# geometrian/simple-spectral

Hardware: AMD Instinct MI355X
Metric: Msamples/s (w*h*spp/s) cornell-srgb 512x512 (higher is better)
Workload: dtype f32

## Files before the change

### simple_spectral_amd/csrc/ssx_api.hip

```cpp
#include "ssx_kernels.hip"
#include "ssx_debug.hip"

#include "../../include/ssx.h"

#include <chrono>
#include <array>
#include <atomic>
#include <cstdarg>
#include <cstdio>
#include <cstdlib>
#include <cmath>
#include <algorithm>
#include <cstring>
#include <mutex>
#include <string>
#include <thread>
#include <vector>

#include <limits.h>
#include <set>

#include "ssx_jit.h"

namespace {
// ... 40 lines not shown
	int n_cus = 0;
	hipStream_t stream = nullptr;
	DeviceBuffer d_blob;
	uint32_t blob_words = 0;
	uint32_t path_blob_words = 0;
	uint32_t topology = 0;
	int jit_mode = SSX_JIT_BACKGROUND;
	const ssx_jit::Kernels* jit_kernels[ssx_jit::kVariants] = {};
	uint32_t libm = SSX_LIBM_BUILD;
	uint32_t variant = SSX_LIBM_BUILD;
	bool jit_pending = false, jit_requested = false;
	ssx_jit::VidTable jit_vid;
	DeviceBuffer d_blob_jit; uint32_t blob_jit_words = 0, path_blob_jit_words = 0;
	uint64_t generic_samples = 0;
	int jit_state = SSX_JIT_STATE_NONE; std::string jit_message;
	std::vector<DeviceBuffer> d_textures;
	DeviceBuffer d_jh_data;
	bool rgb_mode = false;
	bool fuse_resolve = true;
	float calib_frames = 0.0f;
	float calib_left = 0.0f;
	bool pre_hits = false;
	DeviceBuffer d_accum;
	DeviceBuffer d_unit_counter;
	int resident_blocks = 0;
	int gen_blocks = 0;
	uint32_t max_wave_slots = 0;
	uint32_t queue_words = SSX_QUEUE_WORDS_WIDE;
	DeviceBuffer d_samples;
	DeviceBuffer d_logs;
	DeviceBuffer d_out;
	DeviceBuffer d_peer;
	bool have_scene = false;
	bool have_cam_dir = false;

	std::thread worker;
	std::atomic<int> rendering{0};
	std::atomic<int> stop_flag{0};
	std::atomic<uint32_t> done_spp{0};
	std::atomic<uint32_t> done_tiles{0};
	uint32_t total_spp = 0;
	int worker_rc = 0;
	std::atomic<uint64_t> units_enqueued{0};
	ssx_render_params cur{};
	struct SumsState { bool continuable = false, noise_valid = false, spectral_valid = false; uint32_t noise_batches = 0; } sums;
	uint32_t k_begin = 0;
	uint64_t scene_digest = 0;
// ... 66 lines not shown

uint32_t tiles_across(uint32_t pixels) { return (pixels + 7u) / 8u; }
size_t accum_bytes(uint32_t width, uint32_t height) { return (size_t)tiles_across(width) * tiles_across(height) * 64u * 4 * sizeof(double); }
size_t image_bytes(uint32_t width, uint32_t height) { return (size_t)width * height * 4 * sizeof(float); }

SsxPixelGrid pixel_grid(const ssx_render_params* p) {
	const uint32_t tx = tiles_across(p->width);
	return SsxPixelGrid{ p->width, p->height, tx, p->tile_first, p->tile_stride, p->tile_skew % tx };
}
dim3 pixel_blocks(const ssx_render_params* p) { return dim3((p->width * p->height + 255u) / 256u); }

int clear_sums(ssx_ctx* ctx, uint32_t width, uint32_t height, hipStream_t stream) {
	SSX_HIP(ctx, hipMemsetAsync(ctx->d_accum.ptr, 0, accum_bytes(width, height), stream));
	return SSX_OK;
}
void sums_invalidate(ssx_ctx* ctx) { ctx->sums = ssx_ctx::SumsState{}; }
void sums_publish(ssx_ctx* ctx, uint32_t done_spp, int64_t noise_batches = -1) {
	if (noise_batches >= 0) { ctx->sums.noise_valid = true; ctx->sums.noise_batches = (uint32_t)noise_batches; }
	ctx->done_spp.store(done_spp); ctx->sums.continuable = true;
}

constexpr size_t kSampleBufferBudget = (size_t)16 << 30;
size_t bytes_per_sample(const ssx_ctx* ctx) { return ctx->spectral_bins ? SSX_BYTES_PER_SAMPLE_FLUX : SSX_BYTES_PER_SAMPLE; }
constexpr size_t kAuxWordsPer64Records = 5;
size_t bytes_per_64_records(const ssx_ctx* ctx) { return 64u * bytes_per_sample(ctx) + kAuxWordsPer64Records * sizeof(uint32_t); }
size_t sample_bytes(const ssx_ctx* ctx, size_t records) { return records / 64u * bytes_per_64_records(ctx); }
size_t sample_slots(const ssx_ctx* ctx) { return ctx->d_samples.bytes / bytes_per_64_records(ctx) * 64u; }
size_t log_records(const ssx_ctx* ctx) { return ctx->d_logs.bytes / SSX_LOG_BYTES_PER_RECORD; }
constexpr uint32_t kMinUnits = 3072;
constexpr uint64_t kSamplesPerSync = (uint64_t)32 << 20;

struct LaunchPlan { SsxKernelArgs args; uint32_t max_spp_per_launch; };

LaunchPlan make_plan(ssx_ctx* ctx, const ssx_render_params* p, bool ask_device = true) {
	LaunchPlan pl{};
	SsxKernelArgs& a = pl.args;
	a.blob = ctx->d_blob.as<uint32_t>(); a.blob_words = ctx->path_blob_words;
	a.width = p->width; a.height = p->height;
	a.inv_width = 1.0 / (double)p->width; a.inv_height = 1.0 / (double)p->height;
	a.tiles_x = tiles_across(p->width);
	a.n_tiles = a.tiles_x * tiles_across(p->height);
	a.tile_first = p->tile_first; a.tile_stride = p->tile_stride; a.tile_skew = p->tile_skew % a.tiles_x;
	a.indirect_only = p->indirect_only ? 1u : 0u;
	a.no_els = p->no_explicit_light_sampling ? 1u : 0u;
	a.no_flat_field = p->no_flat_field_correction ? 1u : 0u;
	a.seed = p->seed;
	a.rgb_mode = ctx->rgb_mode ? 1u : 0u;
	a.fuse_resolve = ctx->fuse_resolve ? 1u : 0u;
	a.pre_hits = ctx->pre_hits ? 1u : 0u;
	a.my_tiles = a.n_tiles > p->tile_first ? (a.n_tiles - p->tile_first + p->tile_stride - 1u) / p->tile_stride : 0u;
// ... 59 lines not shown
			ctx->stage_ms[k] += ms;
		}
	}
	ctx->ev_used = 0;
	return SSX_OK;
}

int timing_events(ssx_ctx* ctx, hipEvent_t** out) {
	if (ctx->ev_used + 6 > 6 * 64) { int r = collect_timing(ctx); if (r) return r; }
	while (ctx->ev_pool.size() < ctx->ev_used + 6) {
		hipEvent_t e;
		SSX_HIP(ctx, hipEventCreateWithFlags(&e, hipEventDisableSystemFence));
		ctx->ev_pool.push_back(e);
	}
	*out = &ctx->ev_pool[ctx->ev_used];
	ctx->ev_used += 6;
	return SSX_OK;
}

struct Batch { SsxKernelArgs a; uint32_t units; uint64_t n_rec; hipEvent_t* tev; int rc; };

uint32_t unit_spp_of(const ssx_ctx* ctx) { return ctx->calib_frames >= 2.0f ? SSX_MAX_UNIT_KS / 2u : SSX_MAX_UNIT_KS; }

Batch make_batch(ssx_ctx* ctx, const LaunchPlan& pl, uint32_t k0, uint32_t k1) {
	Batch b{};
	b.a = pl.args;
	SsxKernelArgs& a = b.a;
	const uint32_t n_k = k1 - k0;
	a.k0 = k0; a.k1 = k1;
	a.n_records = (uint64_t)a.my_tiles * n_k * 64u;
	uint32_t g = unit_spp_of(ctx);
	while (g > 1u && (uint64_t)((n_k + g - 1u) / g) * a.my_tiles < kMinUnits) g >>= 1;
	a.group_spp = g;
	if (a.group_spp > n_k) a.group_spp = n_k;
	a.unit_cohorts = (a.group_spp + SSX_COHORT_KS - 1u) / SSX_COHORT_KS;
	a.unit_grab = ctx->calib_frames >= 2.0f ? 1u : 4u;
	if (a.unit_grab < 1u || a.unit_grab > 32u || a.group_spp == 0u || a.unit_cohorts == 0u) {
		b.rc = fail(ctx, SSX_ERR_STATE, fmt("internal: launch with unit_grab = %u (1..32), group_spp = %u, unit_cohorts = %u", a.unit_grab, a.group_spp, a.unit_cohorts));
		return b;
	}
	a.n_groups = (n_k + a.group_spp - 1) / a.group_spp;
	b.units = a.my_tiles * a.n_groups;
	b.n_rec = a.n_records;
	b.rc = ensure_logs(ctx, a.unit_cohorts);
	if (b.rc == SSX_OK) bind_arrays(a, ctx->d_samples.as<uint8_t>(), a.n_records, ctx->d_logs.as<uint8_t>(), log_records(ctx), ctx->spectral_bins != 0u);
	a.accum = ctx->d_accum.as<double>();
	uint32_t* const aux = reinterpret_cast<uint32_t*>(ctx->d_samples.as<uint8_t>() + sample_slots(ctx) * bytes_per_sample(ctx));
	a.unit_state = aux;
	a.tile_mask = aux + b.units;
	if (b.rc == SSX_OK && (size_t)a.my_tiles * 4u + b.units > (sample_slots(ctx) / 64u) * kAuxWordsPer64Records) b.rc = fail(ctx, SSX_ERR_STATE, "internal: launch larger than the sample allocation");
	return b;
}

size_t path_lds_bytes(uint32_t blob_words, uint32_t queue_words) {
	size_t n = ((size_t)blob_words + SSX_LDS_PREFIX_WORDS) * 4 + 4u * ((size_t)SSX_QUEUE_ENTRIES * queue_words + SSX_WAVE_COUNTER_WORDS) * 4u;
#ifdef SSX_REGTIME
	n += 4u * SSX_NTIME * 8u;
#endif
	return n;
}
struct PathKernel { const char* name; void (*host)(SsxKernelArgs); };
#define SSX_PK(k) { #k, k }
static const PathKernel kPathKernels[ssx_jit::kVariants][3][2] = {
	{ { SSX_PK(ssx_render_kernel), SSX_PK(ssx_render_kernel_nq) }, { SSX_PK(ssx_render_kernel_cornell), SSX_PK(ssx_render_kernel_cornell_nq) },
	  { SSX_PK(ssx_render_kernel_plane), SSX_PK(ssx_render_kernel_plane_nq) } },
	{ { SSX_PK(ssx_render_kernel_glibc), SSX_PK(ssx_render_kernel_nq_glibc) }, { SSX_PK(ssx_render_kernel_cornell_glibc), SSX_PK(ssx_render_kernel_cornell_nq_glibc) },
	  { SSX_PK(ssx_render_kernel_plane_glibc), SSX_PK(ssx_render_kernel_plane_nq_glibc) } },
	{ { SSX_PK(ssx_render_kernel_flux), SSX_PK(ssx_render_kernel_nq_flux) }, { SSX_PK(ssx_render_kernel_cornell_flux), SSX_PK(ssx_render_kernel_cornell_nq_flux) },
	  { SSX_PK(ssx_render_kernel_plane_flux), SSX_PK(ssx_render_kernel_plane_nq_flux) } } };
#undef SSX_PK
static const char* const kJitKernelNames[2] = { "ssx_render_kernel_jit", "ssx_render_kernel_jit_nq" };
const PathKernel& path_kernel_of(const ssx_ctx* ctx, bool narrow) { return kPathKernels[ctx->variant][ctx->topology < 3u ? ctx->topology : 0u][narrow]; }
// ... 25 lines not shown
	} else {
		void* args[] = { &a };
		SSX_HIP(ctx, hipLaunchKernel(k.host, dim3(blocks), dim3(256), args, lds, stream));
	}
	return SSX_OK;
}
int pick_queue(ssx_ctx* ctx, uint32_t blob_words, uint32_t* queue_words, int* blocks_per_cu) {
	int wide = 0, narrow = 0, rc;
	if (path_lds_bytes(blob_words, SSX_QUEUE_WORDS_WIDE) <= 65536u)
		if ((rc = occupancy_of(ctx, path_kernel_ref(ctx, false), path_lds_bytes(blob_words, SSX_QUEUE_WORDS_WIDE), &wide))) return rc;
	if ((rc = occupancy_of(ctx, path_kernel_ref(ctx, true), path_lds_bytes(blob_words, SSX_QUEUE_WORDS_NARROW), &narrow))) return rc;
	const bool use_narrow = narrow > wide || env_on("SSX_NARROW_QUEUE");
	*queue_words = use_narrow ? SSX_QUEUE_WORDS_NARROW : SSX_QUEUE_WORDS_WIDE;
	if (blocks_per_cu) *blocks_per_cu = use_narrow ? narrow : wide;
	return SSX_OK;
}

bool fuses_generate(const ssx_ctx* ctx, const SsxKernelArgs& a) {
	const char* fuse_env = debug_env("SSX_FUSE_GEN");
	const bool tiles_fit = a.tiles_x <= 0xFFFFu && tiles_across(a.height) <= 0xFFFFu;
	return ctx->topology == 2u && !a.pre_hits && tiles_fit && !(fuse_env && fuse_env[0] == '0');
}

int enqueue_generate(ssx_ctx* ctx, const Batch& b, hipStream_t stream) {
	SsxKernelArgs ga = b.a;
	ga.blob_words = ctx->blob_words;
	if (ga.pre_hits) {
		hipLaunchKernelGGL(ssx_tile_mask_kernel, dim3((ga.my_tiles + 3u) / 4u), dim3(256), 0, stream, ga);
		SSX_HIP(ctx, hipGetLastError());
	}
	const KernelRef gen_kernel{ (const void*)ssx_generate_kernel };
	const size_t gen_lds = ((size_t)ga.blob_words + SSX_LDS_PREFIX_WORDS) * 4;
	if (ctx->gen_blocks == 0) { const int rc = blocks_that_fit(ctx, gen_kernel, gen_lds, &ctx->gen_blocks); if (rc) return rc; }
	const uint64_t want = (b.n_rec + 255u) / 256u;
	return launch_kernel(ctx, gen_kernel, (uint32_t)(want < (uint64_t)ctx->gen_blocks ? want : (uint64_t)ctx->gen_blocks), gen_lds, stream, ga);
}

int enqueue_path(ssx_ctx* ctx, Batch& b, const KernelRef& kernel, uint32_t queue_words, uint32_t blob_words, int resident_blocks, hipStream_t stream) {
	if (!ctx->d_unit_counter.ptr) {
		SSX_HIP(ctx, ctx->d_unit_counter.reserve(4 * sizeof(uint32_t)));
		SSX_HIP(ctx, hipMemsetAsync(ctx->d_unit_counter.ptr, 0, 4 * sizeof(uint32_t), stream));
	}
	b.a.blob_words = blob_words; b.a.queue_words = queue_words;
	SSX_HIP(ctx, hipMemsetAsync(ctx->d_unit_counter.ptr, 0, 2 * sizeof(uint32_t), stream));
	SSX_HIP(ctx, hipMemsetAsync(b.a.unit_state, 0, (size_t)b.units * sizeof(uint32_t), stream));
	b.a.unit_counter = ctx->d_unit_counter.as<uint32_t>();
	const uint32_t want_blocks = (b.units + 3u) / 4u;
	uint32_t blocks = want_blocks < (uint32_t)resident_blocks ? want_blocks : (uint32_t)resident_blocks;
	if (blocks * 4u > ctx->max_wave_slots) blocks = ctx->max_wave_slots / 4u;
	return launch_kernel(ctx, kernel, blocks, path_lds_bytes(blob_words, queue_words), stream, b.a);
}

int launch_batch(ssx_ctx* ctx, Batch& b, hipStream_t stream) {
	if (b.rc) return b.rc;
	int rc;
	if (ctx->timing) { if ((rc = timing_events(ctx, &b.tev))) return rc; SSX_HIP(ctx, hipEventRecord(b.tev[0], stream)); }
	b.a.fuse_gen = fuses_generate(ctx, b.a) ? 1u : 0u;
	if (!b.a.fuse_gen && (rc = enqueue_generate(ctx, b, stream))) return rc;
	if (ctx->timing) SSX_HIP(ctx, hipEventRecord(b.tev[1], stream));
	const bool plan = ctx->resident_blocks == 0;
	if (plan && (rc = pick_queue(ctx, b.a.blob_words, &ctx->queue_words, nullptr))) return rc;
	const KernelRef path_kernel = path_kernel_ref(ctx, ctx->queue_words == SSX_QUEUE_WORDS_NARROW);
	if (plan && (rc = blocks_that_fit(ctx, path_kernel, path_lds_bytes(b.a.blob_words, ctx->queue_words), &ctx->resident_blocks))) return rc;
	if ((rc = enqueue_path(ctx, b, path_kernel, ctx->queue_words, b.a.blob_words, ctx->resident_blocks, stream))) return rc;
	ctx->units_enqueued.fetch_add(b.units);
	if (ctx->timing) for (int k = 2; k < 6; ++k) SSX_HIP(ctx, hipEventRecord(b.tev[k], stream));
	return SSX_OK;
}

constexpr uint64_t kJitAfterSamples = kSamplesPerSync;
void maybe_swap_jit(ssx_ctx* ctx, uint64_t samples) {
	if (!ctx->jit_pending) return;
	std::string err;
	const ssx_jit::Kernels* k = nullptr;
	const ssx_jit::State st = ssx_jit::lookup(ctx->device, ctx->jit_vid, &k, &err, ctx->variant);
	if (st == ssx_jit::State::Ready) {
		std::swap(ctx->d_blob, ctx->d_blob_jit);
		ctx->blob_words = ctx->blob_jit_words; ctx->path_blob_words = ctx->path_blob_jit_words;
		ctx->topology = 3u;
		ctx->jit_kernels[ctx->variant] = k;
		ctx->resident_blocks = 0; ctx->gen_blocks = 0;
		ctx->jit_pending = false; ctx->jit_state = SSX_JIT_STATE_SPECIALISED;
	} else if (st == ssx_jit::State::Failed) {
		ctx->jit_pending = false; ctx->jit_state = SSX_JIT_STATE_FAILED; ctx->jit_message = err;
	} else {
		ctx->generic_samples += samples;
		if (!ctx->jit_requested && ctx->generic_samples >= kJitAfterSamples) { ssx_jit::request(ctx->jit_vid, ctx->variant); ctx->jit_requested = true; }
	}
}

int ensure_libm_kernels(ssx_ctx* ctx, uint32_t libm) {
	const ssx_jit::Kernels*& have = ctx->jit_kernels[libm];
	if (ctx->topology != 3u || have) return SSX_OK;
	std::string err;
	const ssx_jit::Kernels* k = ssx_jit::get(ctx->device, ctx->jit_vid, &err, libm);
	if (!k) return fail(ctx, SSX_ERR_STATE, "the scene's specialised kernels for this libm could not be compiled: " + err);
	have = k;
	return SSX_OK;
}

int ready_to_launch(ssx_ctx* ctx, const ssx_render_params* p, bool need_out) {
	const uint32_t variant = (ctx->spectral_bins && p->libm == SSX_LIBM_BUILD && !ctx->rgb_mode) ? ssx_jit::kVariantFlux : p->libm;
	const int rc = ensure_libm_kernels(ctx, variant);
	if (rc) return rc;
// ... 20 lines not shown

int calibrate(ssx_ctx* ctx) {
	ssx_render_params cp{};
	cp.struct_size = sizeof cp; cp.width = 64; cp.height = 64; cp.spp = 4; cp.tile_stride = 1;
	ctx->fuse_resolve = false;
	ctx->pre_hits = false;
	LaunchPlan pl = make_plan(ctx, &cp);
	int rc = ensure_samples(ctx, pl, cp.spp);
	if (rc) return rc;
	Batch b = make_batch(ctx, pl, 0, cp.spp);
	if (b.rc) return b.rc;
	if ((rc = enqueue_generate(ctx, b, ctx->stream))) return rc;
	const KernelRef kernel{ (const void*)ssx_calibrate_kernel };
	int blocks = 0;
	if ((rc = blocks_that_fit(ctx, kernel, path_lds_bytes(ctx->blob_words, SSX_QUEUE_WORDS_NARROW), &blocks))) return rc;
	if ((rc = enqueue_path(ctx, b, kernel, SSX_QUEUE_WORDS_NARROW, ctx->blob_words, blocks, ctx->stream))) return rc;
	SSX_HIP(ctx, hipStreamSynchronize(ctx->stream));
	std::vector<uint4> recs((size_t)b.n_rec);
	SSX_HIP(ctx, hipMemcpy(recs.data(), b.a.st, recs.size() * sizeof(uint4), hipMemcpyDeviceToHost));
	uint64_t frames = 0;
	for (const uint4& r : recs) frames += (r.y >> 2) & 0xFu;
	ctx->calib_frames = (float)((double)frames / (double)recs.size());
	uint32_t counters[2] = { 0u, 0u };
	SSX_HIP(ctx, hipMemcpy(counters, ctx->d_unit_counter.ptr, sizeof counters, hipMemcpyDeviceToHost));
	ctx->calib_left = (float)((double)counters[1] / (double)recs.size());
	ctx->pre_hits = ctx->calib_left >= 0.3f;
	if (const char* e = debug_env("SSX_PRE_HITS")) { if (e[0] != '\0') ctx->pre_hits = e[0] != '0'; }
	ctx->fuse_resolve = true;
	return ensure_logs(ctx, (unit_spp_of(ctx) + SSX_COHORT_KS - 1u) / SSX_COHORT_KS);
}

int launch_finalize(ssx_ctx* ctx, const ssx_render_params* p, uint32_t spp, float* d_out, hipStream_t stream, uint32_t done_tiles = 0xFFFFFFFFu) {
	hipLaunchKernelGGL(ssx_finalize_kernel, pixel_blocks(p), dim3(256), 0, stream,
	                   ctx->d_accum.as<const double>(), (float4*)d_out, pixel_grid(p), spp, ctx->rgb_mode ? 1u : 0u, done_tiles);
	SSX_HIP(ctx, hipGetLastError());
	return SSX_OK;
}

int noise_begin(ssx_ctx* ctx, const ssx_render_params* p, uint32_t k_begin, bool continuing);
int noise_batch(ssx_ctx* ctx, const ssx_render_params* p, uint32_t n_k, hipStream_t stream);
int spectral_refuses(ssx_ctx* ctx, const ssx_render_params& p, bool tile_walk);
int spectral_begin(ssx_ctx* ctx, uint32_t my_tiles, bool continuing, bool* active);
int spectral_batch(ssx_ctx* ctx, const ssx_render_params* p, const LaunchPlan& pl, uint32_t n_k, hipStream_t stream);

int finish_walk(ssx_ctx* ctx, const ssx_render_params& p, uint32_t spp, uint32_t done_tiles) {
	if (const int rc = launch_finalize(ctx, &p, spp, ctx->d_out.as<float>(), ctx->stream, done_tiles)) return rc;
	SSX_HIP(ctx, hipStreamSynchronize(ctx->stream));
// ... 314 lines not shown
	if (ctx->jit_pending) {
		SSX_HIP(ctx, ctx->d_blob_jit.reserve(blob_jit.size() * 4));
		SSX_HIP(ctx, hipMemcpy(ctx->d_blob_jit.ptr, blob_jit.data(), blob_jit.size() * 4, hipMemcpyHostToDevice));
		const SsxBlobHeader* bh = reinterpret_cast<const SsxBlobHeader*>(blob_jit.data());
		ctx->blob_jit_words = (uint32_t)blob_jit.size(); ctx->path_blob_jit_words = bh->words_without_perm;
	}
	SSX_HIP(ctx, ctx->d_blob.reserve(blob.size() * 4));
	SSX_HIP(ctx, hipMemcpy(ctx->d_blob.ptr, blob.data(), blob.size() * 4, hipMemcpyHostToDevice));
	ctx->blob_words = (uint32_t)blob.size();
	{
		SsxBlobHeader* bh = reinterpret_cast<SsxBlobHeader*>(blob.data());
		ctx->topology = bh->topology;
		ctx->path_blob_words = (bh->topology || bh->perm_hbm) ? bh->words_without_perm : ctx->blob_words;
		if (bh->perm_hbm) {
			const uint64_t at = (uint64_t)(uintptr_t)(ctx->d_blob.as<uint32_t>() + bh->off_perm);
			bh->perm_ptr_lo = (uint32_t)at; bh->perm_ptr_hi = (uint32_t)(at >> 32);
			SSX_HIP(ctx, hipMemcpy(ctx->d_blob.ptr, blob.data(), sizeof(SsxBlobHeader), hipMemcpyHostToDevice));
			ctx->blob_words = bh->words_without_perm;
		}
	}
	ctx->have_cam_dir = have_cam_dir;
	ctx->lambda_min = s->lambda_min; ctx->lambda_step = s->lambda_step;
	ctx->resident_blocks = 0; ctx->gen_blocks = 0;
	ctx->have_scene = true;
	ctx->scene_digest = scene_digest_of(s);
	return calibrate(ctx);
}

static uint32_t device_batch(const ssx_render_params* p, const LaunchPlan& pl) {
	uint32_t batch = p->spp_per_launch ? p->spp_per_launch : p->spp;
	if (batch > p->spp) batch = p->spp;
	if (batch > pl.max_spp_per_launch) {
		const uint32_t n = (p->spp + pl.max_spp_per_launch - 1u) / pl.max_spp_per_launch;
		batch = (p->spp + n - 1u) / n;
	}
	return batch;
}

int ssx_render_device(ssx_ctx* ctx, const ssx_render_params* p_in, void* d_xyza_out, void* hip_stream) {
	if (!ctx) return SSX_ERR_ARG;
	ssx_render_params pp;
	int rc = take_params(ctx, p_in, &pp);
	if (rc) return rc;
	const ssx_render_params* const p = &pp;
	if (!d_xyza_out) return fail(ctx, SSX_ERR_ARG, "d_xyza_out is NULL");
	if (ctx->spectral_bins) return fail(ctx, SSX_ERR_ARG, "spectral output is on (ssx_set_spectral_bins): ssx_render_device does not bin its samples; use ssx_render_start");
// ... 253 lines not shown
	const std::string text = ssx_jit::pass1_source(name, t);
	copy_text(text, out, out_size);
	return (int)text.size();
}

int ssx_calibration_info(ssx_ctx* ctx, float* frames_per_sample, float* rays_left_per_sample, int* camera_rays_pretraced) {
	if (!ctx) return SSX_ERR_ARG;
	if (!ctx->have_scene) return fail(ctx, SSX_ERR_STATE, "no scene uploaded");
	if (frames_per_sample) *frames_per_sample = ctx->calib_frames;
	if (rays_left_per_sample) *rays_left_per_sample = ctx->calib_left;
	if (camera_rays_pretraced) *camera_rays_pretraced = ctx->pre_hits ? 1 : 0;
	return SSX_OK;
}

int ssx_scratch_info(ssx_ctx* ctx, uint64_t* sample_bytes, uint64_t* log_bytes) {
	if (!ctx) return SSX_ERR_ARG;
	if (sample_bytes) *sample_bytes = (uint64_t)sample_slots(ctx) * bytes_per_sample(ctx);
	if (log_bytes) *log_bytes = (uint64_t)ctx->d_logs.bytes;
	return SSX_OK;
}

int ssx_sums_info(ssx_ctx* ctx, uint64_t* units_parked, uint64_t* units_chained) {
	if (!ctx) return SSX_ERR_ARG;
	uint32_t c[4] = { 0u, 0u, 0u, 0u };
	if (ctx->d_unit_counter.ptr) {
		SSX_HIP(ctx, hipSetDevice(ctx->device));
		const int rc = wait_device_pending(ctx);
		if (rc) return rc;
		SSX_HIP(ctx, hipMemcpy(c, ctx->d_unit_counter.ptr, sizeof c, hipMemcpyDeviceToHost));
	}
	if (units_parked) *units_parked = c[2];
	if (units_chained) *units_chained = c[3];
	return SSX_OK;
}

int ssx_units_info(ssx_ctx* ctx, uint64_t* units_enqueued) {
	if (!ctx) return SSX_ERR_ARG;
	if (units_enqueued) *units_enqueued = ctx->units_enqueued.load();
	return SSX_OK;
}

int ssx_kernel_variant(ssx_ctx* ctx) { return (ctx && ctx->have_scene) ? (int)ctx->topology : -1; }

const char* ssx_kernel_name(ssx_ctx* ctx) {
	if (!ctx || !ctx->have_scene) return nullptr;
	if (hipSetDevice(ctx->device) != hipSuccess) return nullptr;
	uint32_t qw = 0;
	if (pick_queue(ctx, ctx->path_blob_words, &qw, nullptr) != SSX_OK) return nullptr;
	const bool narrow = qw == SSX_QUEUE_WORDS_NARROW;
	return ctx->topology == 3u ? kJitKernelNames[narrow] : path_kernel_of(ctx, narrow).name;
}

int ssx_plan_info(ssx_ctx* ctx, float* frames_per_sample, int* fold_in_path_kernel) {
	if (!ctx) return SSX_ERR_ARG;
	if (!ctx->have_scene) return fail(ctx, SSX_ERR_STATE, "no scene uploaded");
// ... 32 lines not shown
```

### simple_spectral_amd/csrc/ssx_blob.h

```cpp
#pragma once
#include <stdint.h>
#include <hip/hip_runtime.h>

#define SSX_QUEUE_ENTRIES 128u
#define SSX_QUEUE_WORDS_WIDE 12u
#define SSX_QUEUE_WORDS_NARROW 8u
#define SSX_LDS_PREFIX_WORDS 80u
#define SSX_BLOB_MAX_BYTES 48576u

#define SSX_PERM_COUNT 3u
#define SSX_PERM_WORDS_PER_QUAD (SSX_PERM_COUNT * 12u)
#define SSX_PERM_AXES { { 1u, 2u }, { 0u, 2u }, { 0u, 1u } }

struct SsxBlobSpectrum {
	uint32_t offset;
	uint32_t n;
	float low, delta_recip;
};

struct SsxBlobQuad {
	float pos[4][3];
	float st[4][2];
	float normal[2][3];
	uint32_t kind;
// ... 67 lines not shown
	uint32_t no_els;
	uint32_t my_tiles;
	uint32_t group_spp;
	uint32_t n_groups;
	uint64_t seed;
	float4* ray;
	uint4* st;
	float4* hit;
	uint8_t* logs;
	uint32_t log_cap;
	uint64_t n_records;
	uint32_t* unit_counter;
	uint32_t rgb_mode;
	uint32_t fuse_resolve;
	uint32_t unit_cohorts;
	double* accum;
	uint32_t* tile_mask;
	uint32_t* unit_state;
	uint32_t no_flat_field;
	uint32_t keep_samples;
	uint32_t pre_hits;
	uint32_t queue_words;
	uint32_t unit_grab;
	uint32_t pad_grab_;
	double inv_width, inv_height;
	uint32_t fuse_gen;
	float4* flux;
};
```

### simple_spectral_amd/csrc/ssx_kernels.hip

```cpp
#include <hip/hip_runtime.h>
#ifndef __HIPCC_RTC__
#include <stdint.h>
#endif

#include "ssx_blob.h"
#include "ssx_exact.h"
#include "ssx_lanestat.h"
extern __shared__ __attribute__((aligned(16))) uint32_t ssx_lds[];
#define SSX_FM_TABLE (reinterpret_cast<const double*>(ssx_lds))
#ifdef SSX_JIT_BUILD
#include "ssx_fmath.h"
#else
#include "../../include/ssx_fmath.h"
#endif
#define SSX_GM_TABLE (SSX_FM_TABLE + SSX_FM_I_A11)
#ifdef SSX_JIT_BUILD
#include "ssx_glibc_math.h"
#else
#include "../../include/ssx_glibc_math.h"
#endif
__device__ const double ssx_fm_coeff_values[SSX_FM_N_COEFF] = SSX_FM_COEFF_INIT;
__device__ const double ssx_gm_coeff_values[SSX_GM_N_COEFF] = SSX_GM_COEFF_INIT;
static_assert(2 * SSX_FM_N_COEFF <= SSX_LDS_PREFIX_WORDS, "coefficient table");
static_assert(SSX_FM_I_A11 + SSX_GM_N_COEFF <= SSX_FM_N_COEFF, "glibc coefficients in the arc-cosine slots");
// ... 1118 lines not shown
		bool keep = false;
		if (q < h.n_quads) {
			keep = true;
#pragma unroll
			for (int k = 0; k < 4; ++k) {
				bool all_out = true;
#pragma unroll
				for (int v = 0; v < 4; ++v) {
					const double vx = (double)quads[q].pos[v][0] - (double)h.cam_pos[0], vy = (double)quads[q].pos[v][1] - (double)h.cam_pos[1], vz = (double)quads[q].pos[v][2] - (double)h.cam_pos[2];
					const double dist = __builtin_sqrt(vx * vx + vy * vy + vz * vz);
					const double sd = n[k][0] * vx + n[k][1] * vy + n[k][2] * vz;
					all_out = all_out && (sd < -1.0e-4 * dist);
				}
				if (all_out) keep = false;
			}
		}
		const uint64_t m = __ballot(keep);
		if (lane == 0u) { a.tile_mask[4u * slot + 2u * g] = (uint32_t)m; a.tile_mask[4u * slot + 2u * g + 1u] = (uint32_t)(m >> 32); }
	}
}
#endif

struct WorkUnit {
	uint32_t slot, grp;
	uint32_t tile;
	uint32_t txy;
	uint32_t dims;
	__device__ __forceinline__ uint32_t tw() const { return dims & 15u; }
	__device__ __forceinline__ uint32_t th() const { return (dims >> 4) & 15u; }
	__device__ __forceinline__ uint32_t n_kq() const { return dims >> 8; }
	__device__ __forceinline__ uint32_t npx() const { return tw() * th(); }
	__device__ __forceinline__ uint32_t n_items() const { return npx() * n_kq(); }
	__device__ __forceinline__ uint32_t k_off(const SsxKernelArgs& a) const { return grp * a.group_spp; }
	__device__ __forceinline__ uint32_t rec_base(const SsxKernelArgs& a) const { return (slot * (a.k1 - a.k0) + grp * a.group_spp) * 64u; }
};
__device__ __forceinline__ void unit_setup(const SsxKernelArgs& hot, uint32_t unit, WorkUnit& u) {
	(void)hot;
	const __attribute__((address_space(4))) SsxKernelArgs& a = cold_args();
	const uint32_t slot = unit % a.my_tiles, grp = unit / a.my_tiles;
	uint32_t tx, ty;
	const uint32_t tile = tile_of_slot(a, slot, tx, ty);
	const uint32_t ka = a.k0 + grp * a.group_spp;
	const uint32_t kb = min(ka + a.group_spp, a.k1);
	u.dims = min(8u, a.width - tx * 8u) | (min(8u, a.height - ty * 8u) << 4) | ((kb - ka) << 8);
	u.slot = slot; u.grp = grp;
	u.tile = tile; u.txy = tx | (ty << 16);
}
__device__ __forceinline__ void sums_release(uint32_t* cnt) {
#ifdef SSX_ACCUM_FORMAL
	wave_release(cnt);
	wave_acquire(cnt);
#else
	(void)cnt;
	__builtin_amdgcn_fence(__ATOMIC_RELEASE, "workgroup");
	asm volatile("s_waitcnt vmcnt(0)" ::: "memory");
#endif
}
__device__ __forceinline__ void sums_acquire(uint32_t* cnt) {
#ifdef SSX_ACCUM_FORMAL
	wave_release(cnt);
	wave_acquire(cnt);
#else
	(void)cnt;
	__builtin_amdgcn_fence(__ATOMIC_ACQUIRE, "workgroup");
#endif
}
#ifdef SSX_ACCUM_FORMAL
#define SSX_SUMS_ACQ __ATOMIC_ACQUIRE
#define SSX_SUMS_ACQ_REL __ATOMIC_ACQ_REL
#else
#define SSX_SUMS_ACQ __ATOMIC_RELAXED
#define SSX_SUMS_ACQ_REL __ATOMIC_RELAXED
#endif
__device__ __forceinline__ void sums_chain(uint32_t slot, uint32_t grp, uint32_t lane, uint32_t* cnt) {
	const __attribute__((address_space(4))) SsxKernelArgs& a = cold_args();
	uint32_t tx, ty;
	const uint32_t tile = tile_of_slot(a, slot, tx, ty);
	const bool has_px = (lane & 7u) < min(8u, a.width - tx * 8u) && (lane >> 3) < min(8u, a.height - ty * 8u);
	double* const px = a.accum + (size_t)tile * 256u + lane;
	uint32_t* state = a.unit_state + (slot * a.n_groups + grp);
	uint32_t rec_at = (slot * (a.k1 - a.k0) + grp * a.group_spp) * 64u;
	double acc[4] = { 0.0, 0.0, 0.0, 0.0 };
	if (has_px) { acc[0] = ld_agent(px); acc[1] = ld_agent(px + 64); acc[2] = ld_agent(px + 128); acc[3] = ld_agent(px + 192); }
	for (;;) {
		const uint32_t n = min(a.group_spp, (a.k1 - a.k0) - grp * a.group_spp);
		if (has_px) {
			for (uint32_t kq = 0; kq < n; ++kq) add_staged_sample(a.rgb_mode != 0u, acc, a.ray + (rec_at + kq * 64u + lane));
			st_agent(px, acc[0]); st_agent(px + 64, acc[1]); st_agent(px + 128, acc[2]); st_agent(px + 192, acc[3]);
		}
		if (++grp >= a.n_groups) return;
		sums_release(cnt);
		++state; rec_at += a.group_spp * 64u;
		uint32_t was = 0u;
		if (lane == 0u) was = __hip_atomic_fetch_or(state, SSX_UNIT_TURN, SSX_SUMS_ACQ_REL, __HIP_MEMORY_SCOPE_AGENT);
		was = (uint32_t)__builtin_amdgcn_readfirstlane((int)was);
		sums_acquire(cnt);
		if (was != SSX_UNIT_PARKED) return;
		if (lane == 0u) atomicAdd(a.unit_counter + 3, 1u);
	}
}
template <bool NARROW, bool FLUX = false>
__device__ __forceinline__ void unit_fold(const Lds& L, const SsxKernelArgs& a, const WorkUnit& u, uint32_t wave_slot, uint32_t tag, uint32_t* cnt) {
	wave_acquire(cnt);
	__builtin_amdgcn_fence(__ATOMIC_RELEASE, "workgroup");
	__builtin_amdgcn_fence(__ATOMIC_ACQUIRE, "agent");
	const uint32_t lane = threadIdx.x & 63u;
	const bool has_px = (lane & 7u) < u.tw() && (lane >> 3) < u.th();
	const __attribute__((address_space(4))) SsxKernelArgs& c = cold_args();
	uint32_t* const state = c.unit_state + (u.slot * c.n_groups + u.grp);
	double* const px = c.accum + (size_t)u.tile * 256u + lane;
	bool mine = true;
	if (u.grp) {
		mine = ((uint32_t)__builtin_amdgcn_readfirstlane((int)__hip_atomic_load(state, SSX_SUMS_ACQ, __HIP_MEMORY_SCOPE_AGENT)) & SSX_UNIT_TURN) != 0u;
		sums_acquire(cnt);
	}
	double acc[4] = { 0.0, 0.0, 0.0, 0.0 };
	if (mine && has_px) { acc[0] = ld_agent(px); acc[1] = ld_agent(px + 64); acc[2] = ld_agent(px + 128); acc[3] = ld_agent(px + 192); }
	if (has_px)
		for (uint32_t kq = 0, n_kq = u.n_kq(), rec_base = u.rec_base(a); kq < n_kq; kq += SSX_COHORT_KS) {
			const uint32_t log_rec = log_region(a, wave_slot, tag, kq / SSX_COHORT_KS);
			resolve_records<SSX_COHORT_KS, NARROW, FLUX>(L, a, rec_base + kq * 64u + lane, 64u, min(SSX_COHORT_KS, n_kq - kq), log_rec * SSX_MAX_FRAMES, log_rec * SSX_MAX_LEVELS, lane, acc, !mine);
		}
	if (mine) {
		if (has_px) { st_agent(px, acc[0]); st_agent(px + 64, acc[1]); st_agent(px + 128, acc[2]); st_agent(px + 192, acc[3]); }
		if (u.grp + 1u >= c.n_groups) return;
		sums_release(cnt);
		uint32_t was = 0u;
		if (lane == 0u) was = __hip_atomic_fetch_or(state + 1, SSX_UNIT_TURN, SSX_SUMS_ACQ_REL, __HIP_MEMORY_SCOPE_AGENT);
		was = (uint32_t)__builtin_amdgcn_readfirstlane((int)was);
		sums_acquire(cnt);
		if (was != SSX_UNIT_PARKED) return;
		if (lane == 0u) atomicAdd(c.unit_counter + 3, 1u);
		sums_chain(u.slot, u.grp + 1u, lane, cnt);
	} else {
		sums_release(cnt);
		uint32_t was = 0u;
		if (lane == 0u) {
			atomicAdd(c.unit_counter + 2, 1u);
			uint32_t expected = 0u;
			(void)__hip_atomic_compare_exchange_strong(state, &expected, SSX_UNIT_PARKED, SSX_SUMS_ACQ_REL, SSX_SUMS_ACQ, __HIP_MEMORY_SCOPE_AGENT);
			was = expected;
		}
		was = (uint32_t)__builtin_amdgcn_readfirstlane((int)was);
		sums_acquire(cnt);
		if (was == SSX_UNIT_TURN) sums_chain(u.slot, u.grp, lane, cnt);
	}
}

template <int TOPO, bool NARROW, bool CALIB = false, bool GLIBC = false, bool FLUX = false>
__device__ __forceinline__ void render_body(const SsxKernelArgs& a) {
	constexpr bool FUSE_GEN = TOPO == 2;
	uint32_t* const lds_words = stage_lds<GLIBC>(a);
	Lds L; L.w = lds_words;

	const uint32_t wave = (uint32_t)__builtin_amdgcn_readfirstlane((int)(threadIdx.x >> 6)), lane = threadIdx.x & 63u;
	const uint32_t wave_slot = blockIdx.x * 4u + wave;
	const SsxBlobHeader& hg = *reinterpret_cast<const SsxBlobHeader*>(a.blob);
	const V3 cam = mk(hg.cam_pos[0], hg.cam_pos[1], hg.cam_pos[2]);

	Path p;
	p.orig = mk(0.0f, 0.0f, 0.0f); p.dir = mk(0.0f, 0.0f, 1.0f); p.ignore = -1; p.depth = 0; p.rec_index = 0; p.lambda_0 = 0.0f; p.prev_slot = SSX_NO_SLOT;
	p.hit_tri = 0; p.hit_dist = 0.0f; p.hit_st_x = p.hit_st_y = 0.0f;
	p.rng.state = 0; p.rng.inc = 1;
	bool active = false;
	uint32_t p_tag = 0;
	constexpr uint32_t queue_words = SSX_QUEUE_ENTRIES * (NARROW ? SSX_QUEUE_WORDS_NARROW : SSX_QUEUE_WORDS_WIDE);
	uint32_t* const log_cnt = lds_words + a.blob_words + 4u * queue_words + wave * SSX_WAVE_COUNTER_WORDS;
	SsxTimer tm;
// ... 12 lines not shown
	uint32_t grab = 0;
	auto end_path = [&](uint32_t level_word, uint32_t hit_anything) {
		const uint32_t tail = hit_anything | ((level_word >> 26) << 1) | (p.depth << 2) | (p.prev_slot << 6) | ((level_word >> 13) << 19);
		a.st[p.rec_index] = make_uint4(__float_as_uint(p.lambda_0), tail, (uint32_t)p.rng.state, (uint32_t)(p.rng.state >> 32));
		wave_release(log_cnt);
		active = false;
	};
	auto refill = [&](bool with_hit) {
		const uint32_t n_items = cur.n_items();
		if (!(cur_valid && next_item < n_items)) return;
		const uint64_t idle = __ballot(!active);
		if (!active) {
			const uint32_t item = next_item + __builtin_amdgcn_mbcnt_hi((uint32_t)(idle >> 32), __builtin_amdgcn_mbcnt_lo((uint32_t)idle, 0u));
			if (item < n_items) {
				SSX_STAT(19);
				uint32_t in_tile, kq;
				const uint32_t npx = cur.npx(), tw = cur.tw();
				if (npx == 64u) { in_tile = item & 63u; kq = item >> 6; }
				else { const uint32_t r = item % npx; kq = item / npx; in_tile = (r / tw) * 8u + r % tw; }
				p.rec_index = cur.rec_base(a) + kq * 64u + in_tile;
				float4 ray; uint4 st;
				if (FUSE_GEN && a.fuse_gen) {
					const __attribute__((address_space(4))) SsxKernelArgs& c = cold_args();
					generate_sample(L.hdr(), c, (cur.txy & 0xFFFFu) * 8u + (in_tile & 7u), (cur.txy >> 16) * 8u + (in_tile >> 3), c.k0 + cur.grp * c.group_spp + kq, ray, st);
					if (c.no_flat_field) c.ray[p.rec_index] = ray;
				} else {
					ray = a.ray[p.rec_index];
					st = a.st[p.rec_index];
				}
				p.dir = mk(ray.x, ray.y, ray.z);
				p.lambda_0 = ray.w;
				p.rng.state = ((uint64_t)st.y << 32) | st.x;
				p.rng.inc = ((uint64_t)st.w << 32) | st.z;
				p.orig = cam;
				p.ignore = -1;
				p.depth = 0;
				p.prev_slot = SSX_NO_SLOT;
				const uint32_t cohort = kq / SSX_COHORT_KS;
				p_tag = cohort | (cur_tag << 2) | ((cur_tag * a.unit_cohorts + cohort) << 3) | ((kq % SSX_COHORT_KS) << 8);
				active = true;
				if (with_hit) {
					const float4 ht = a.hit[p.rec_index];
					p.hit_dist = ht.x; p.hit_st_x = ht.y; p.hit_st_y = ht.z; p.hit_tri = __float_as_int(ht.w);
					active = p.hit_tri >= 0;
				}
			}
		}
// ... 160 lines not shown
```

Before: 3177.

## Grade work-unit sizes toward the end of each batch and cache tile mask

```diff
diff --git a/simple_spectral_amd/csrc/ssx_api.hip b/simple_spectral_amd/csrc/ssx_api.hip
--- a/simple_spectral_amd/csrc/ssx_api.hip
+++ b/simple_spectral_amd/csrc/ssx_api.hip
@@ -86,7 +86,9 @@
 	float calib_left = 0.0f;
 	bool pre_hits = false;
 	DeviceBuffer d_accum;
-	DeviceBuffer d_unit_counter;
+	DeviceBuffer d_unit_stats;
+	DeviceBuffer d_tile_mask;
+	struct TileMaskKey { uint32_t valid, width, height, tile_first, tile_stride, tile_skew; const void* blob; } tile_mask_key{};
 	int resident_blocks = 0;
 	int gen_blocks = 0;
 	uint32_t max_wave_slots = 0;
@@ -199,10 +201,13 @@
 
 constexpr size_t kSampleBufferBudget = (size_t)16 << 30;
 size_t bytes_per_sample(const ssx_ctx* ctx) { return ctx->spectral_bins ? SSX_BYTES_PER_SAMPLE_FLUX : SSX_BYTES_PER_SAMPLE; }
-constexpr size_t kAuxWordsPer64Records = 5;
+constexpr size_t kAuxWordsPer64Records = 5, kAuxFixedWords = 4;
 size_t bytes_per_64_records(const ssx_ctx* ctx) { return 64u * bytes_per_sample(ctx) + kAuxWordsPer64Records * sizeof(uint32_t); }
-size_t sample_bytes(const ssx_ctx* ctx, size_t records) { return records / 64u * bytes_per_64_records(ctx); }
-size_t sample_slots(const ssx_ctx* ctx) { return ctx->d_samples.bytes / bytes_per_64_records(ctx) * 64u; }
+size_t sample_bytes(const ssx_ctx* ctx, size_t records) { return records / 64u * bytes_per_64_records(ctx) + kAuxFixedWords * sizeof(uint32_t); }
+size_t sample_slots(const ssx_ctx* ctx) {
+	const size_t fixed = kAuxFixedWords * sizeof(uint32_t);
+	return ctx->d_samples.bytes < fixed ? 0u : (ctx->d_samples.bytes - fixed) / bytes_per_64_records(ctx) * 64u;
+}
 size_t log_records(const ssx_ctx* ctx) { return ctx->d_logs.bytes / SSX_LOG_BYTES_PER_RECORD; }
 constexpr uint32_t kMinUnits = 3072;
 constexpr uint64_t kSamplesPerSync = (uint64_t)32 << 20;
@@ -308,6 +313,28 @@
 
 uint32_t unit_spp_of(const ssx_ctx* ctx) { return ctx->calib_frames >= 2.0f ? SSX_MAX_UNIT_KS / 2u : SSX_MAX_UNIT_KS; }
 
+void grade_units(const ssx_ctx* ctx, SsxKernelArgs& a, uint32_t n_k) {
+	uint32_t g = a.group_spp;
+	const uint64_t tiles = a.my_tiles ? a.my_tiles : 1u;
+	uint32_t fine = (uint32_t)std::min<uint64_t>((4u * (uint64_t)ctx->max_wave_slots + tiles - 1u) / tiles, 65536u), mid = 2u * fine;
+	bool grade = g > 2u && (uint64_t)fine + mid + g <= n_k;
+	if (const char* e = debug_env("SSX_UNIT_GRADING")) {
+		unsigned eg = 0, em = 0, ef = 0;
+		if (sscanf(e, "%u,%u,%u", &eg, &em, &ef) == 3 && eg >= 1u && eg <= SSX_MAX_UNIT_KS) {
+			g = std::min(eg, n_k); mid = std::min(em, n_k) & ~1u; fine = std::min(ef, n_k);
+			grade = g > 1u && (uint64_t)fine + mid + g <= n_k && fine + mid > 0u;
+		}
+	}
+	a.group_spp = g;
+	a.k_mid = a.k_fine = n_k;
+	if (grade) {
+		a.k_mid = (n_k - fine - mid) / g * g;
+		a.k_fine = n_k - fine - ((n_k - a.k_mid - fine) & 1u);
+	}
+	a.g_mid = (a.k_mid + g - 1u) / g;
+	a.n_groups = a.g_mid + (a.k_fine - a.k_mid) / 2u + (n_k - a.k_fine);
+}
+
 Batch make_batch(ssx_ctx* ctx, const LaunchPlan& pl, uint32_t k0, uint32_t k1) {
 	Batch b{};
 	b.a = pl.args;
@@ -319,21 +346,22 @@
 	while (g > 1u && (uint64_t)((n_k + g - 1u) / g) * a.my_tiles < kMinUnits) g >>= 1;
 	a.group_spp = g;
 	if (a.group_spp > n_k) a.group_spp = n_k;
+	grade_units(ctx, a, n_k);
 	a.unit_cohorts = (a.group_spp + SSX_COHORT_KS - 1u) / SSX_COHORT_KS;
 	a.unit_grab = ctx->calib_frames >= 2.0f ? 1u : 4u;
-	if (a.unit_grab < 1u || a.unit_grab > 32u || a.group_spp == 0u || a.unit_cohorts == 0u) {
-		b.rc = fail(ctx, SSX_ERR_STATE, fmt("internal: launch with unit_grab = %u (1..32), group_spp = %u, unit_cohorts = %u", a.unit_grab, a.group_spp, a.unit_cohorts));
+	if (a.unit_grab < 1u || a.unit_grab > 32u || a.group_spp == 0u || a.group_spp > SSX_MAX_UNIT_KS || a.unit_cohorts == 0u || n_k > 65536u) {
+		b.rc = fail(ctx, SSX_ERR_STATE, fmt("internal: launch with unit_grab = %u (1..32), group_spp = %u, unit_cohorts = %u, %u samples per pixel", a.unit_grab, a.group_spp, a.unit_cohorts, n_k));
 		return b;
 	}
-	a.n_groups = (n_k + a.group_spp - 1) / a.group_spp;
 	b.units = a.my_tiles * a.n_groups;
 	b.n_rec = a.n_records;
 	b.rc = ensure_logs(ctx, a.unit_cohorts);
 	if (b.rc == SSX_OK) bind_arrays(a, ctx->d_samples.as<uint8_t>(), a.n_records, ctx->d_logs.as<uint8_t>(), log_records(ctx), ctx->spectral_bins != 0u);
 	a.accum = ctx->d_accum.as<double>();
 	uint32_t* const aux = reinterpret_cast<uint32_t*>(ctx->d_samples.as<uint8_t>() + sample_slots(ctx) * bytes_per_sample(ctx));
-	a.unit_state = aux;
-	a.tile_mask = aux + b.units;
+	a.unit_counter = aux;
+	a.unit_state = aux + kAuxFixedWords;
+	a.tile_mask = a.unit_state + b.units;
 	if (b.rc == SSX_OK && (size_t)a.my_tiles * 4u + b.units > (sample_slots(ctx) / 64u) * kAuxWordsPer64Records) b.rc = fail(ctx, SSX_ERR_STATE, "internal: launch larger than the sample allocation");
 	return b;
 }
@@ -405,13 +433,30 @@
 	return ctx->topology == 2u && !a.pre_hits && tiles_fit && !(fuse_env && fuse_env[0] == '0');
 }
 
+int ensure_tile_mask(ssx_ctx* ctx, SsxKernelArgs& ga, hipStream_t stream) {
+	hipStreamCaptureStatus capture = hipStreamCaptureStatusNone;
+	(void)hipStreamIsCapturing(stream, &capture);
+	const bool cached = capture != hipStreamCaptureStatusActive;
+	const ssx_ctx::TileMaskKey key{ 1u, ga.width, ga.height, ga.tile_first, ga.tile_stride, ga.tile_skew, ga.blob };
+	if (cached) {
+		ssx_ctx::TileMaskKey& have = ctx->tile_mask_key;
+		const bool same = have.valid && have.width == key.width && have.height == key.height && have.tile_first == key.tile_first &&
+		                  have.tile_stride == key.tile_stride && have.tile_skew == key.tile_skew && have.blob == key.blob;
+		if (same) { ga.tile_mask = ctx->d_tile_mask.as<uint32_t>(); return SSX_OK; }
+		have.valid = 0u;
+		SSX_HIP(ctx, ctx->d_tile_mask.reserve((size_t)ga.my_tiles * 4u * sizeof(uint32_t)));
+		ga.tile_mask = ctx->d_tile_mask.as<uint32_t>();
+	}
+	hipLaunchKernelGGL(ssx_tile_mask_kernel, dim3((ga.my_tiles + 3u) / 4u), dim3(256), 0, stream, ga);
+	SSX_HIP(ctx, hipGetLastError());
+	if (cached) ctx->tile_mask_key = key;
+	return SSX_OK;
+}
+
 int enqueue_generate(ssx_ctx* ctx, const Batch& b, hipStream_t stream) {
 	SsxKernelArgs ga = b.a;
 	ga.blob_words = ctx->blob_words;
-	if (ga.pre_hits) {
-		hipLaunchKernelGGL(ssx_tile_mask_kernel, dim3((ga.my_tiles + 3u) / 4u), dim3(256), 0, stream, ga);
-		SSX_HIP(ctx, hipGetLastError());
-	}
+	if (ga.pre_hits) { const int rc = ensure_tile_mask(ctx, ga, stream); if (rc) return rc; }
 	const KernelRef gen_kernel{ (const void*)ssx_generate_kernel };
 	const size_t gen_lds = ((size_t)ga.blob_words + SSX_LDS_PREFIX_WORDS) * 4;
 	if (ctx->gen_blocks == 0) { const int rc = blocks_that_fit(ctx, gen_kernel, gen_lds, &ctx->gen_blocks); if (rc) return rc; }
@@ -420,14 +465,13 @@
 }
 
 int enqueue_path(ssx_ctx* ctx, Batch& b, const KernelRef& kernel, uint32_t queue_words, uint32_t blob_words, int resident_blocks, hipStream_t stream) {
-	if (!ctx->d_unit_counter.ptr) {
-		SSX_HIP(ctx, ctx->d_unit_counter.reserve(4 * sizeof(uint32_t)));
-		SSX_HIP(ctx, hipMemsetAsync(ctx->d_unit_counter.ptr, 0, 4 * sizeof(uint32_t), stream));
+	if (!ctx->d_unit_stats.ptr) {
+		SSX_HIP(ctx, ctx->d_unit_stats.reserve(2 * sizeof(uint32_t)));
+		SSX_HIP(ctx, hipMemsetAsync(ctx->d_unit_stats.ptr, 0, 2 * sizeof(uint32_t), stream));
 	}
 	b.a.blob_words = blob_words; b.a.queue_words = queue_words;
-	SSX_HIP(ctx, hipMemsetAsync(ctx->d_unit_counter.ptr, 0, 2 * sizeof(uint32_t), stream));
-	SSX_HIP(ctx, hipMemsetAsync(b.a.unit_state, 0, (size_t)b.units * sizeof(uint32_t), stream));
-	b.a.unit_counter = ctx->d_unit_counter.as<uint32_t>();
+	b.a.unit_stats = ctx->d_unit_stats.as<uint32_t>();
+	SSX_HIP(ctx, hipMemsetAsync(b.a.unit_counter, 0, (kAuxFixedWords + (size_t)b.units) * sizeof(uint32_t), stream));
 	const uint32_t want_blocks = (b.units + 3u) / 4u;
 	uint32_t blocks = want_blocks < (uint32_t)resident_blocks ? want_blocks : (uint32_t)resident_blocks;
 	if (blocks * 4u > ctx->max_wave_slots) blocks = ctx->max_wave_slots / 4u;
@@ -463,6 +507,7 @@
 		ctx->topology = 3u;
 		ctx->jit_kernels[ctx->variant] = k;
 		ctx->resident_blocks = 0; ctx->gen_blocks = 0;
+		ctx->tile_mask_key.valid = 0u;
 		ctx->jit_pending = false; ctx->jit_state = SSX_JIT_STATE_SPECIALISED;
 	} else if (st == ssx_jit::State::Failed) {
 		ctx->jit_pending = false; ctx->jit_state = SSX_JIT_STATE_FAILED; ctx->jit_message = err;
@@ -529,7 +574,7 @@
 	for (const uint4& r : recs) frames += (r.y >> 2) & 0xFu;
 	ctx->calib_frames = (float)((double)frames / (double)recs.size());
 	uint32_t counters[2] = { 0u, 0u };
-	SSX_HIP(ctx, hipMemcpy(counters, ctx->d_unit_counter.ptr, sizeof counters, hipMemcpyDeviceToHost));
+	SSX_HIP(ctx, hipMemcpy(counters, b.a.unit_counter, sizeof counters, hipMemcpyDeviceToHost));
 	ctx->calib_left = (float)((double)counters[1] / (double)recs.size());
 	ctx->pre_hits = ctx->calib_left >= 0.3f;
 	if (const char* e = debug_env("SSX_PRE_HITS")) { if (e[0] != '\0') ctx->pre_hits = e[0] != '0'; }
@@ -890,6 +935,7 @@
 	ctx->have_cam_dir = have_cam_dir;
 	ctx->lambda_min = s->lambda_min; ctx->lambda_step = s->lambda_step;
 	ctx->resident_blocks = 0; ctx->gen_blocks = 0;
+	ctx->tile_mask_key.valid = 0u;
 	ctx->have_scene = true;
 	ctx->scene_digest = scene_digest_of(s);
 	return calibrate(ctx);
@@ -1189,15 +1235,15 @@
 
 int ssx_sums_info(ssx_ctx* ctx, uint64_t* units_parked, uint64_t* units_chained) {
 	if (!ctx) return SSX_ERR_ARG;
-	uint32_t c[4] = { 0u, 0u, 0u, 0u };
-	if (ctx->d_unit_counter.ptr) {
+	uint32_t c[2] = { 0u, 0u };
+	if (ctx->d_unit_stats.ptr) {
 		SSX_HIP(ctx, hipSetDevice(ctx->device));
 		const int rc = wait_device_pending(ctx);
 		if (rc) return rc;
-		SSX_HIP(ctx, hipMemcpy(c, ctx->d_unit_counter.ptr, sizeof c, hipMemcpyDeviceToHost));
-	}
-	if (units_parked) *units_parked = c[2];
-	if (units_chained) *units_chained = c[3];
+		SSX_HIP(ctx, hipMemcpy(c, ctx->d_unit_stats.ptr, sizeof c, hipMemcpyDeviceToHost));
+	}
+	if (units_parked) *units_parked = c[0];
+	if (units_chained) *units_chained = c[1];
 	return SSX_OK;
 }
 
diff --git a/simple_spectral_amd/csrc/ssx_blob.h b/simple_spectral_amd/csrc/ssx_blob.h
--- a/simple_spectral_amd/csrc/ssx_blob.h
+++ b/simple_spectral_amd/csrc/ssx_blob.h
@@ -113,8 +113,12 @@
 	uint32_t pre_hits;
 	uint32_t queue_words;
 	uint32_t unit_grab;
-	uint32_t pad_grab_;
+	uint32_t k_mid;
 	double inv_width, inv_height;
 	uint32_t fuse_gen;
+	uint32_t k_fine;
 	float4* flux;
+	uint32_t* unit_stats;
+	uint32_t g_mid;
+	uint32_t pad_end_;
 };
diff --git a/simple_spectral_amd/csrc/ssx_kernels.hip b/simple_spectral_amd/csrc/ssx_kernels.hip
--- a/simple_spectral_amd/csrc/ssx_kernels.hip
+++ b/simple_spectral_amd/csrc/ssx_kernels.hip
@@ -1164,7 +1164,8 @@
 #endif
 
 struct WorkUnit {
-	uint32_t slot, grp;
+	uint32_t slot;
+	uint32_t kg;
 	uint32_t tile;
 	uint32_t txy;
 	uint32_t dims;
@@ -1173,19 +1174,29 @@
 	__device__ __forceinline__ uint32_t n_kq() const { return dims >> 8; }
 	__device__ __forceinline__ uint32_t npx() const { return tw() * th(); }
 	__device__ __forceinline__ uint32_t n_items() const { return npx() * n_kq(); }
-	__device__ __forceinline__ uint32_t k_off(const SsxKernelArgs& a) const { return grp * a.group_spp; }
-	__device__ __forceinline__ uint32_t rec_base(const SsxKernelArgs& a) const { return (slot * (a.k1 - a.k0) + grp * a.group_spp) * 64u; }
+	__device__ __forceinline__ uint32_t k_off() const { return kg & 0xFFFFu; }
+	__device__ __forceinline__ uint32_t grp() const { return kg >> 16; }
+	__device__ __forceinline__ uint32_t rec_base(const SsxKernelArgs& a) const { return (slot * (a.k1 - a.k0) + k_off()) * 64u; }
 };
+template <typename Args>
+__device__ __forceinline__ void unit_span(const Args& a, uint32_t grp, uint32_t& k_off, uint32_t& n_kq) {
+	if (grp < a.g_mid) { k_off = grp * a.group_spp; n_kq = min(a.group_spp, a.k_mid - k_off); }
+	else {
+		const uint32_t g_fine = a.g_mid + ((a.k_fine - a.k_mid) >> 1);
+		if (grp < g_fine) { k_off = a.k_mid + (grp - a.g_mid) * 2u; n_kq = 2u; }
+		else { k_off = a.k_fine + (grp - g_fine); n_kq = 1u; }
+	}
+}
 __device__ __forceinline__ void unit_setup(const SsxKernelArgs& hot, uint32_t unit, WorkUnit& u) {
 	(void)hot;
 	const __attribute__((address_space(4))) SsxKernelArgs& a = cold_args();
 	const uint32_t slot = unit % a.my_tiles, grp = unit / a.my_tiles;
 	uint32_t tx, ty;
 	const uint32_t tile = tile_of_slot(a, slot, tx, ty);
-	const uint32_t ka = a.k0 + grp * a.group_spp;
-	const uint32_t kb = min(ka + a.group_spp, a.k1);
-	u.dims = min(8u, a.width - tx * 8u) | (min(8u, a.height - ty * 8u) << 4) | ((kb - ka) << 8);
-	u.slot = slot; u.grp = grp;
+	uint32_t k_off, n_kq;
+	unit_span(a, grp, k_off, n_kq);
+	u.dims = min(8u, a.width - tx * 8u) | (min(8u, a.height - ty * 8u) << 4) | (n_kq << 8);
+	u.slot = slot; u.kg = k_off | (grp << 16);
 	u.tile = tile; u.txy = tx | (ty << 16);
 }
 __device__ __forceinline__ void sums_release(uint32_t* cnt) {
@@ -1221,24 +1232,25 @@
 	const bool has_px = (lane & 7u) < min(8u, a.width - tx * 8u) && (lane >> 3) < min(8u, a.height - ty * 8u);
 	double* const px = a.accum + (size_t)tile * 256u + lane;
 	uint32_t* state = a.unit_state + (slot * a.n_groups + grp);
-	uint32_t rec_at = (slot * (a.k1 - a.k0) + grp * a.group_spp) * 64u;
 	double acc[4] = { 0.0, 0.0, 0.0, 0.0 };
 	if (has_px) { acc[0] = ld_agent(px); acc[1] = ld_agent(px + 64); acc[2] = ld_agent(px + 128); acc[3] = ld_agent(px + 192); }
 	for (;;) {
-		const uint32_t n = min(a.group_spp, (a.k1 - a.k0) - grp * a.group_spp);
+		uint32_t k_off, n;
+		unit_span(a, grp, k_off, n);
+		const uint32_t rec_at = (slot * (a.k1 - a.k0) + k_off) * 64u;
 		if (has_px) {
 			for (uint32_t kq = 0; kq < n; ++kq) add_staged_sample(a.rgb_mode != 0u, acc, a.ray + (rec_at + kq * 64u + lane));
 			st_agent(px, acc[0]); st_agent(px + 64, acc[1]); st_agent(px + 128, acc[2]); st_agent(px + 192, acc[3]);
 		}
 		if (++grp >= a.n_groups) return;
 		sums_release(cnt);
-		++state; rec_at += a.group_spp * 64u;
+		++state;
 		uint32_t was = 0u;
 		if (lane == 0u) was = __hip_atomic_fetch_or(state, SSX_UNIT_TURN, SSX_SUMS_ACQ_REL, __HIP_MEMORY_SCOPE_AGENT);
 		was = (uint32_t)__builtin_amdgcn_readfirstlane((int)was);
 		sums_acquire(cnt);
 		if (was != SSX_UNIT_PARKED) return;
-		if (lane == 0u) atomicAdd(a.unit_counter + 3, 1u);
+		if (lane == 0u) atomicAdd(a.unit_stats + 1, 1u);
 	}
 }
 template <bool NARROW, bool FLUX = false>
@@ -1249,10 +1261,10 @@
 	const uint32_t lane = threadIdx.x & 63u;
 	const bool has_px = (lane & 7u) < u.tw() && (lane >> 3) < u.th();
 	const __attribute__((address_space(4))) SsxKernelArgs& c = cold_args();
-	uint32_t* const state = c.unit_state + (u.slot * c.n_groups + u.grp);
+	uint32_t* const state = c.unit_state + (u.slot * c.n_groups + u.grp());
 	double* const px = c.accum + (size_t)u.tile * 256u + lane;
 	bool mine = true;
-	if (u.grp) {
+	if (u.grp()) {
 		mine = ((uint32_t)__builtin_amdgcn_readfirstlane((int)__hip_atomic_load(state, SSX_SUMS_ACQ, __HIP_MEMORY_SCOPE_AGENT)) & SSX_UNIT_TURN) != 0u;
 		sums_acquire(cnt);
 	}
@@ -1265,27 +1277,27 @@
 		}
 	if (mine) {
 		if (has_px) { st_agent(px, acc[0]); st_agent(px + 64, acc[1]); st_agent(px + 128, acc[2]); st_agent(px + 192, acc[3]); }
-		if (u.grp + 1u >= c.n_groups) return;
+		if (u.grp() + 1u >= c.n_groups) return;
 		sums_release(cnt);
 		uint32_t was = 0u;
 		if (lane == 0u) was = __hip_atomic_fetch_or(state + 1, SSX_UNIT_TURN, SSX_SUMS_ACQ_REL, __HIP_MEMORY_SCOPE_AGENT);
 		was = (uint32_t)__builtin_amdgcn_readfirstlane((int)was);
 		sums_acquire(cnt);
 		if (was != SSX_UNIT_PARKED) return;
-		if (lane == 0u) atomicAdd(c.unit_counter + 3, 1u);
-		sums_chain(u.slot, u.grp + 1u, lane, cnt);
+		if (lane == 0u) atomicAdd(c.unit_stats + 1, 1u);
+		sums_chain(u.slot, u.grp() + 1u, lane, cnt);
 	} else {
 		sums_release(cnt);
 		uint32_t was = 0u;
 		if (lane == 0u) {
-			atomicAdd(c.unit_counter + 2, 1u);
+			atomicAdd(c.unit_stats, 1u);
 			uint32_t expected = 0u;
 			(void)__hip_atomic_compare_exchange_strong(state, &expected, SSX_UNIT_PARKED, SSX_SUMS_ACQ_REL, SSX_SUMS_ACQ, __HIP_MEMORY_SCOPE_AGENT);
 			was = expected;
 		}
 		was = (uint32_t)__builtin_amdgcn_readfirstlane((int)was);
 		sums_acquire(cnt);
-		if (was == SSX_UNIT_TURN) sums_chain(u.slot, u.grp, lane, cnt);
+		if (was == SSX_UNIT_TURN) sums_chain(u.slot, u.grp(), lane, cnt);
 	}
 }
 
@@ -1344,7 +1356,7 @@
 				float4 ray; uint4 st;
 				if (FUSE_GEN && a.fuse_gen) {
 					const __attribute__((address_space(4))) SsxKernelArgs& c = cold_args();
-					generate_sample(L.hdr(), c, (cur.txy & 0xFFFFu) * 8u + (in_tile & 7u), (cur.txy >> 16) * 8u + (in_tile >> 3), c.k0 + cur.grp * c.group_spp + kq, ray, st);
+					generate_sample(L.hdr(), c, (cur.txy & 0xFFFFu) * 8u + (in_tile & 7u), (cur.txy >> 16) * 8u + (in_tile >> 3), c.k0 + cur.k_off() + kq, ray, st);
 					if (c.no_flat_field) c.ray[p.rec_index] = ray;
 				} else {
 					ray = a.ray[p.rec_index];
```

New measurement: 3190 (median of 6 runs). About the same (+0.4%).
